# simonmeister/UnFlow

Measured on NVIDIA H100. Metric: frame-pairs/s at 384x1280 FlowNetC, higher is better.
Workload: dtype f32

## Files before the change

unflow_b200/csrc/tc_wgrad.cu:

```cuda
#include "tc_common.cuh"

namespace unflow {
namespace tcw {

using namespace unflow::tc;

constexpr int NTHREADS = 384;
constexpr int KP = 32;

struct WgradParams {
  int N, Hp, Wp;
  int TW, TH, TN;
  int tiles_x, tiles_y, tiles_n;
  int n_ptiles, kc, n_chunks;
  int R, C;
  int cgroups, vgroups;
  int r_blocks, c_blocks, taps, kw;
  int chunk;
  long long *dbg;
  int stride, stride_x, pad_t, pad_l;
  float *dw;
  long long pitch_r, pitch_t;
};

template <int BN>
struct Cfg {
  static constexpr int G_BYTES = BN * KP * 4;
  static constexpr int A_HI = 0;
  static constexpr int A_LO = A_HI + A_BYTES;
  static constexpr int B_HI = A_LO + A_BYTES;
  static constexpr int B_LO = B_HI + G_BYTES;
  static constexpr int SPLIT_BYTES = B_LO + G_BYTES;
  static constexpr int SPLIT_STAGES = 2;
  static constexpr int G_RAW = A_BYTES;
  static constexpr int RAW_BYTES = A_BYTES + G_BYTES;
  static constexpr int RAW0 = SPLIT_STAGES * SPLIT_BYTES;
  static constexpr int FIXED = RAW0 + 1024  + 256 ;
  static constexpr int RAW_STAGES = (SMEM_LIMIT - FIXED) / RAW_BYTES < 8 ? (SMEM_LIMIT - FIXED) / RAW_BYTES : 8;
  static constexpr int SMEM_BYTES = FIXED + RAW_STAGES * RAW_BYTES;
  static_assert(RAW_STAGES >= 3, "TMA at least two K blocks ahead of the split");
  static_assert(SMEM_BYTES <= SMEM_LIMIT, "over the shared memory of a block");
  static_assert(8 * (2 * RAW_STAGES + SPLIT_STAGES) <= 256, "barriers");
};

struct Item {
  int chunk, rb, cb;
};
__device__ __forceinline__ Item decode_item(const WgradParams &p, int it) {
  Item w;
  w.cb = it % p.c_blocks; it /= p.c_blocks;
  w.rb = it % p.r_blocks; it /= p.r_blocks;
  w.chunk = it;
  return w;
}
__device__ __forceinline__ int chunk_len(const WgradParams &p, int chunk) {
  const int k0 = chunk * p.kc;
  return (k0 + p.kc <= p.n_ptiles) ? p.kc : p.n_ptiles - k0;
}

template <int ROWS>
__device__ __forceinline__ void split_transpose(const float *raw, unsigned char *hi, unsigned char *lo, int row0, int ct) {
#pragma unroll
  for (int j = 0; j < ROWS * 8 / 128; ++j) {
    const int i = ct + 128 * j;
    const int r = row0 + i % ROWS, c = i / ROWS;
    const float *src = raw + (r >> 5) * 1024 + (4 * c) * 32 + (r & 31);
    const float4 v = make_float4(src[0], src[32], src[64], src[96]), h = tf32_hi4(v);
    const unsigned o = sw128_offset(r, 4 * c);
    *reinterpret_cast<float4 *>(hi + o) = h;
    *reinterpret_cast<float4 *>(lo + o) = sub4(v, h);
  }
}

template <int BN>
__global__ void __launch_bounds__(NTHREADS, 1)
tc_wgrad_kernel(const __grid_constant__ CUtensorMap mapP, const __grid_constant__ CUtensorMap mapG,
                const __grid_constant__ WgradParams p) {
  using C = Cfg<BN>;
  constexpr int R = BN / 2;
  constexpr int GROUPS = BN / 32;
  extern __shared__ unsigned char smem_raw[];
  const unsigned base = (s32(smem_raw) + 1023u) & ~1023u;
  unsigned char *gbase = smem_raw + (base - s32(smem_raw));
  const unsigned bars = base + C::RAW0 + C::RAW_STAGES * C::RAW_BYTES;
  auto raw_full = [&](int s) { return bars + 8u * s; };
  auto raw_empty = [&](int s) { return bars + 8u * (C::RAW_STAGES + s); };
  auto split_empty = [&](int s) { return bars + 8u * (2 * C::RAW_STAGES + s); };

  const int warp = __shfl_sync(0xffffffffu, threadIdx.x >> 5, 0), lane = threadIdx.x & 31;
  const int total_items = p.n_chunks * p.r_blocks * p.c_blocks;

  if (threadIdx.x == 0) {
    for (int s = 0; s < C::RAW_STAGES; ++s) {
      mbar_init(raw_full(s), 1);
      mbar_init(raw_empty(s), 8);
    }
    for (int s = 0; s < C::SPLIT_STAGES; ++s) mbar_init(split_empty(s), 8);
    asm volatile("fence.mbarrier_init.release.cluster;" ::: "memory");
    asm volatile("prefetch.tensormap [%0];" ::"l"(&mapP) : "memory");
    asm volatile("prefetch.tensormap [%0];" ::"l"(&mapG) : "memory");
  }
  __syncthreads();

  if (warp == 0) {
    int s = 0;
    unsigned ph = 0;
    long long t_wait = 0, t_all = clock64();
    for (int item = blockIdx.x; item < total_items; item += gridDim.x) {
      const Item w = decode_item(p, item);
      int gch[GROUPS], gdx[GROUPS], gdy[GROUPS];
#pragma unroll
      for (int j = 0; j < GROUPS; ++j) {
        const int v = w.cb * GROUPS + j;
        if (v < p.vgroups) {
          const int tap = v / p.cgroups, ky = tap / p.kw;
          gch[j] = (v - tap * p.cgroups) * 32; gdy[j] = ky - p.pad_t; gdx[j] = tap - ky * p.kw - p.pad_l;
        } else {
          gch[j] = p.cgroups * 32; gdx[j] = gdy[j] = 0;
        }
      }
      const int k0 = w.chunk * p.kc, klen = chunk_len(p, w.chunk);
      for (int kb = k0; kb < k0 + klen; ++kb) {
        int q = kb;
        const int px = (q % p.tiles_x) * p.TW; q /= p.tiles_x;
        const int py = (q % p.tiles_y) * p.TH; q /= p.tiles_y;
        const int pn = q * p.TN;
        { const long long t0 = clock64(); mbar_wait(raw_empty(s), ph ^ 1u); t_wait += clock64() - t0; }
        const unsigned st = base + C::RAW0 + s * C::RAW_BYTES;
        if (elect_one()) {
          mbar_expect_tx(raw_full(s), (unsigned)C::RAW_BYTES);
#pragma unroll
          for (int j = 0; j < BM / 32; ++j)
            tma_4d(st + j * 4096, &mapP, raw_full(s), w.rb * BM + 32 * j, px, py, pn);
#pragma unroll
          for (int j = 0; j < GROUPS; ++j)
            tma_4d(st + C::G_RAW + j * 4096, &mapG, raw_full(s), gch[j], p.stride_x * px + gdx[j],
                   p.stride * py + gdy[j], pn);
        }
        __syncwarp();
        if (++s == C::RAW_STAGES) { s = 0; ph ^= 1u; }
      }
    }
    if (p.dbg && blockIdx.x == 0 && lane == 0) { p.dbg[0] = t_wait; p.dbg[1] = clock64() - t_all; }
  } else if (warp >= 4) {
    const int cw = (warp >> 2) - 1;
    const int ct = threadIdx.x - 128 * (cw + 1);
    const int row0 = 64 * cw + 16 * (ct >> 5) + (lane >> 2);
    const int col0 = 2 * (lane & 3);
    unsigned n = 0;
    unsigned t_wait = 0, t_split = 0;
    const unsigned t_all = (unsigned)clock();
    auto split = [&](bool rows) {
      const unsigned rs = n % C::RAW_STAGES, rph = (n / C::RAW_STAGES) & 1u;
      const unsigned ss = n % C::SPLIT_STAGES, sph = (n / C::SPLIT_STAGES) & 1u;
      { const unsigned t0 = (unsigned)clock(); mbar_wait(raw_full(rs), rph); t_wait += (unsigned)clock() - t0; }
      { const unsigned t0 = (unsigned)clock(); mbar_wait(split_empty(ss), sph ^ 1u); t_split += (unsigned)clock() - t0; }
      const float *raw = reinterpret_cast<const float *>(gbase + C::RAW0 + rs * C::RAW_BYTES);
      unsigned char *sp = gbase + ss * C::SPLIT_BYTES;
      if (rows) split_transpose<64>(raw, sp + C::A_HI, sp + C::A_LO, 64 * cw, ct);
      split_transpose<BN / 2>(raw + C::G_RAW / 4, sp + C::B_HI, sp + C::B_LO, cw * (BN / 2), ct);
      __syncwarp();
      if (lane == 0) mbar_arrive(raw_empty(rs));
      fence_proxy_async();
      named_bar_sync(1, 256);
    };
    float sum[R], acc[R];
    for (int item = blockIdx.x; item < total_items; item += gridDim.x) {
      const Item w = decode_item(p, item);
      const int iters = chunk_len(p, w.chunk);
      if (w.rb * BM + 64 * cw >= p.R) {
        for (int it = 0; it < iters; ++it) {
          split(false);
          if (lane == 0) mbar_arrive(split_empty(n % C::SPLIT_STAGES));
          ++n;
        }
        continue;
      }
#pragma unroll
      for (int c = 0; c < R; ++c) sum[c] = 0.f;
      for (int c0 = 0; c0 < iters; c0 += p.chunk) {
        const int c1 = c0 + p.chunk < iters ? c0 + p.chunk : iters;
        for (int it = c0; it < c1; ++it) {
          split(true);
          const unsigned st = base + (n % C::SPLIT_STAGES) * C::SPLIT_BYTES;
          const unsigned long long a_hi = wgmma_desc_k128(st + C::A_HI + cw * (A_BYTES / 2));
          const unsigned long long a_lo = wgmma_desc_k128(st + C::A_LO + cw * (A_BYTES / 2));
          const unsigned long long b_hi = wgmma_desc_k128(st + C::B_HI), b_lo = wgmma_desc_k128(st + C::B_LO);
          fence_regs(acc);
          wgmma_fence();
#pragma unroll
          for (int k = 0; k < KP / 8; ++k) {
            const unsigned long long adv = (unsigned long long)(2 * k);
            Wgmma<BN>::mma(acc, a_lo + adv, b_hi + adv, (it - c0 | k) != 0);
            Wgmma<BN>::mma(acc, a_hi + adv, b_lo + adv, 1);
            Wgmma<BN>::mma(acc, a_hi + adv, b_hi + adv, 1);
          }
          wgmma_commit();
          wgmma_wait<1>();
          fence_regs(acc);
          __syncwarp();
          if (it > c0 && lane == 0) mbar_arrive(split_empty((n - 1) % C::SPLIT_STAGES));
          ++n;
        }
        wgmma_wait<0>();
        fence_regs(acc);
        __syncwarp();
        if (lane == 0) mbar_arrive(split_empty((n - 1) % C::SPLIT_STAGES));
#pragma unroll
        for (int c = 0; c < R; ++c) sum[c] += acc[c];
      }
#pragma unroll
      for (int h = 0; h < 2; ++h) {
        const int r = w.rb * BM + row0 + 8 * h;
        if (r >= p.R) continue;
#pragma unroll
        for (int j = 0; j < BN / 8; ++j) {
          const int col = 8 * j + col0;
          const int v = w.cb * GROUPS + col / 32;
          if (v >= p.vgroups) continue;
          const int tap = v / p.cgroups, c = (v - tap * p.cgroups) * 32 + (col & 31);
          float *dst = p.dw + (long long)r * p.pitch_r + (long long)tap * p.pitch_t + c;
          if (c < p.C) red_add_f32(dst, sum[4 * j + 2 * h]);
          if (c + 1 < p.C) red_add_f32(dst + 1, sum[4 * j + 2 * h + 1]);
        }
      }
    }
    if (p.dbg && blockIdx.x == 0 && threadIdx.x == 128) {
      p.dbg[2] = t_wait; p.dbg[3] = (unsigned)clock() - t_all; p.dbg[4] = t_split;
      p.dbg[5] = C::RAW_STAGES; p.dbg[6] = C::SPLIT_STAGES;
    }
  }
}

template <int BN>
static int launch(const CUtensorMap &mP, const CUtensorMap &mG, const WgradParams &p, cudaStream_t stream) {
  using C = Cfg<BN>;
  static bool attr_set = false;
  if (!attr_set) {
    cudaError_t e = cudaFuncSetAttribute(tc_wgrad_kernel<BN>, cudaFuncAttributeMaxDynamicSharedMemorySize, C::SMEM_BYTES);
    if (e != cudaSuccess) { set_error("tc_wgrad: cannot opt in to %d bytes of shared memory: %s", C::SMEM_BYTES, cudaGetErrorString(e)); return UNFLOW_ECUDA; }
    attr_set = true;
  }
  const long long total = (long long)p.n_chunks * p.r_blocks * p.c_blocks;
  const int grid = total < kNumSMs ? (int)total : kNumSMs;
  tc_wgrad_kernel<BN><<<grid, NTHREADS, C::SMEM_BYTES, stream>>>(mP, mG, p);
  count_launch();
  return check_launch("tc_wgrad_kernel");
}

static int launch_bn(int BN, const CUtensorMap &mP, const CUtensorMap &mG, const WgradParams &p, cudaStream_t stream) {
  if (BN == 128) return launch<128>(mP, mG, p, stream);
  if (BN == 64) return launch<64>(mP, mG, p, stream);
  return launch<32>(mP, mG, p, stream);
}

static void choose_box(WgradParams &p) {
  long long best = -1;
  for (int TW = 1; TW <= 32; TW *= 2)
    for (int TH = 1; TW * TH <= 32; TH *= 2) {
      const int TN = 32 / (TW * TH);
      const long long tiles = (long long)((p.Wp + TW - 1) / TW) * ((p.Hp + TH - 1) / TH) * ((p.N + TN - 1) / TN);
      if (best < 0 || tiles < best || (tiles == best && TW > p.TW)) {
        best = tiles; p.TW = TW; p.TH = TH; p.TN = TN;
      }
    }
  p.tiles_x = (p.Wp + p.TW - 1) / p.TW; p.tiles_y = (p.Hp + p.TH - 1) / p.TH; p.tiles_n = (p.N + p.TN - 1) / p.TN;
  p.n_ptiles = p.tiles_x * p.tiles_y * p.tiles_n;
}

static int make_plan(WgradParams &p, int &BN, int N, int Hp, int Wp, int R, int C, int stride, int kh, int kw,
                     int pad_t, int pad_l) {
  UNFLOW_REQUIRE(N > 0 && Hp > 0 && Wp > 0 && R > 0 && C > 0, "tc_wgrad: bad extents");
  UNFLOW_REQUIRE(stride == 1 || stride == 2, "tc_wgrad: stride must be 1 or 2");
  UNFLOW_REQUIRE(kh > 0 && kw > 0 && kh * kw <= 64, "tc_wgrad: at most 64 taps");
  p.N = N; p.Hp = Hp; p.Wp = Wp; p.R = R; p.C = C; p.chunk = g_chunk; p.dbg = g_dbg;
  p.taps = kh * kw; p.kw = kw; p.stride = p.stride_x = stride; p.pad_t = pad_t; p.pad_l = pad_l;
  choose_box(p);
  p.cgroups = (C + 31) / 32; p.vgroups = p.taps * p.cgroups;
  BN = p.vgroups >= 4 ? 128 : (p.vgroups >= 2 ? 64 : 32);
  p.r_blocks = (R + BM - 1) / BM; p.c_blocks = (p.vgroups + BN / 32 - 1) / (BN / 32);
  const long long tiles = (long long)p.r_blocks * p.c_blocks;
  long long want = (6ll * kNumSMs + tiles - 1) / tiles;
  if (want < 1) want = 1;
  int kc = (int)((p.n_ptiles + want - 1) / want);
  if (kc < 8) kc = p.n_ptiles < 8 ? p.n_ptiles : 8;
  p.kc = kc; p.n_chunks = (p.n_ptiles + kc - 1) / kc;
  UNFLOW_REQUIRE(tiles * p.n_chunks < (1ll << 30), "tc_wgrad: too many work items");
  return UNFLOW_OK;
}

}
}

using namespace unflow;

extern "C" int unflow_tc_wgrad_plan(int N, int Hp, int Wp, int R, int C, int stride, int kh, int kw, int pad_t,
                                    int pad_l, int *out) {
  tcw::WgradParams p{};
  int BN = 0;
  if (tcw::make_plan(p, BN, N, Hp, Wp, R, C, stride, kh, kw, pad_t, pad_l) || !out) return -1;
  const int v[15] = {p.TW, p.TH, p.TN, p.tiles_x, p.tiles_y, p.tiles_n, p.n_ptiles, p.kc, p.n_chunks, p.r_blocks,
                     p.c_blocks, BN, p.taps, p.cgroups, p.vgroups};
  for (int i = 0; i < 15; ++i) out[i] = v[i];
  return 15;
}

extern "C" int unflow_tc_wgrad(const float *P, int N, int Hp, int Wp, int R, long long p_pitch, const float *G,
                               int Hg, int Wg, int C, long long g_pitch, float *dw, long long pitch_r,
                               long long pitch_t, int stride, int kh, int kw, int pad_t, int pad_l, void *stream) {
  UNFLOW_REQUIRE(P && G && dw, "tc_wgrad: null pointer");
  UNFLOW_REQUIRE(Hg > 0 && Wg > 0, "tc_wgrad: bad extents");
  UNFLOW_REQUIRE(p_pitch % 4 == 0 && g_pitch % 4 == 0 && p_pitch >= R && g_pitch >= C,
                 "tc_wgrad: channel pitches must be multiples of 4 floats");
  UNFLOW_REQUIRE(((uintptr_t)P & 15) == 0 && ((uintptr_t)G & 15) == 0, "tc_wgrad: P and G must be 16-byte aligned");
  tcw::WgradParams p{};
  int BN = 0;
  int rc = tcw::make_plan(p, BN, N, Hp, Wp, R, C, stride, kh, kw, pad_t, pad_l);
  if (rc) return rc;
  p.dw = dw; p.pitch_r = pitch_r; p.pitch_t = pitch_t;
  CUtensorMap mP, mG;
  {
    cuuint64_t dims[4] = {(cuuint64_t)R, (cuuint64_t)Wp, (cuuint64_t)Hp, (cuuint64_t)N};
    cuuint64_t strides[3] = {(cuuint64_t)p_pitch * 4, (cuuint64_t)p_pitch * 4 * Wp, (cuuint64_t)p_pitch * 4 * Wp * Hp};
    cuuint32_t box[4] = {32, (cuuint32_t)p.TW, (cuuint32_t)p.TH, (cuuint32_t)p.TN};
    cuuint32_t estr[4] = {1, 1, 1, 1};
    rc = tc::encode(&mP, P, 4, dims, strides, box, estr, CU_TENSOR_MAP_SWIZZLE_NONE);
    if (rc) return rc;
  }
  {
    cuuint64_t dims[4] = {(cuuint64_t)C, (cuuint64_t)Wg, (cuuint64_t)Hg, (cuuint64_t)N};
    cuuint64_t strides[3] = {(cuuint64_t)g_pitch * 4, (cuuint64_t)g_pitch * 4 * Wg, (cuuint64_t)g_pitch * 4 * Wg * Hg};
    cuuint32_t box[4] = {32, (cuuint32_t)(p.TW * stride), (cuuint32_t)(p.TH * stride), (cuuint32_t)p.TN};
    cuuint32_t estr[4] = {1, (cuuint32_t)stride, (cuuint32_t)stride, 1};
    rc = tc::encode(&mG, G, 4, dims, strides, box, estr, CU_TENSOR_MAP_SWIZZLE_NONE);
    if (rc) return rc;
  }
  return tcw::launch_bn(BN, mP, mG, p, (cudaStream_t)stream);
}

extern "C" int unflow_tc_wgrad_window(const float *P, int N, int Ho, int Wo, int R, long long p_pitch,
                                      const float *xp, int H, int Wp, int Cp, float *dw, int kh, int stride,
                                      int pad_t, void *stream) {
  UNFLOW_REQUIRE(P && xp && dw, "tc_wgrad_window: null pointer");
  UNFLOW_REQUIRE(Cp == 4 || Cp == 8 || Cp == 16, "tc_wgrad_window: padded channel count must be 4, 8 or 16");
  UNFLOW_REQUIRE(p_pitch % 4 == 0 && p_pitch >= R, "tc_wgrad_window: bad pitch");
  UNFLOW_REQUIRE(((uintptr_t)P & 15) == 0 && ((uintptr_t)xp & 15) == 0, "tc_wgrad_window: pointers must be 16-byte aligned");
  UNFLOW_REQUIRE(H > 0 && Wp >= stride * (Wo - 1) + 8, "tc_wgrad_window: the padded row must hold the last 8-pixel window");
  const int win = 8 * Cp;
  tcw::WgradParams p{};
  int BN = 0;
  int rc = tcw::make_plan(p, BN, N, Ho, Wo, R, win, stride, kh, 1, pad_t, 0);
  if (rc) return rc;
  p.stride_x = 1;
  p.dw = dw; p.pitch_r = (long long)kh * win; p.pitch_t = win;
  CUtensorMap mP, mG;
  {
    cuuint64_t dims[4] = {(cuuint64_t)R, (cuuint64_t)Wo, (cuuint64_t)Ho, (cuuint64_t)N};
    cuuint64_t strides[3] = {(cuuint64_t)p_pitch * 4, (cuuint64_t)p_pitch * 4 * Wo, (cuuint64_t)p_pitch * 4 * Wo * Ho};
    cuuint32_t box[4] = {32, (cuuint32_t)p.TW, (cuuint32_t)p.TH, (cuuint32_t)p.TN};
    cuuint32_t estr[4] = {1, 1, 1, 1};
    rc = tc::encode(&mP, P, 4, dims, strides, box, estr, CU_TENSOR_MAP_SWIZZLE_NONE);
    if (rc) return rc;
  }
  {
    cuuint64_t dims[4] = {(cuuint64_t)win, (cuuint64_t)Wo, (cuuint64_t)H, (cuuint64_t)N};
    cuuint64_t strides[3] = {(cuuint64_t)stride * Cp * 4, (cuuint64_t)Wp * Cp * 4, (cuuint64_t)Wp * Cp * 4 * H};
    cuuint32_t box[4] = {32, (cuuint32_t)p.TW, (cuuint32_t)(p.TH * stride), (cuuint32_t)p.TN};
    cuuint32_t estr[4] = {1, 1, (cuuint32_t)stride, 1};
    rc = tc::encode(&mG, xp, 4, dims, strides, box, estr, CU_TENSOR_MAP_SWIZZLE_NONE);
    if (rc) return rc;
  }
  return tcw::launch_bn(BN, mP, mG, p, (cudaStream_t)stream);
}
```

Before: 114.8.

## Feed wgrad A operand from registers instead of split shared-memory tiles

The A (P) operand of the 3xTF32 weight-gradient WGMMA is now loaded directly from the swizzled raw TMA stage into registers, split into hi/lo in registers, and issued as register-source wgmma, removing the A split/transpose pass and its shared-memory stage. Raw-stage release moves to after the register loads, and commits are per K-step with double-buffered fragment sets so loads overlap the previous MMAs. Register budgets are rebalanced with setmaxnreg (producer warps shrink, consumers grow), and the P tensor map uses the default swizzle to match the new addressing. This risks register pressure and more per-element conversion work in the consumer warps, and the B-side indexing change must stay consistent with the G layout.

```diff
diff --git a/unflow_b200/csrc/tc_wgrad.cu b/unflow_b200/csrc/tc_wgrad.cu
--- a/unflow_b200/csrc/tc_wgrad.cu
+++ b/unflow_b200/csrc/tc_wgrad.cu
@@ -26,9 +26,7 @@
 template <int BN>
 struct Cfg {
   static constexpr int G_BYTES = BN * KP * 4;
-  static constexpr int A_HI = 0;
-  static constexpr int A_LO = A_HI + A_BYTES;
-  static constexpr int B_HI = A_LO + A_BYTES;
+  static constexpr int B_HI = 0;
   static constexpr int B_LO = B_HI + G_BYTES;
   static constexpr int SPLIT_BYTES = B_LO + G_BYTES;
   static constexpr int SPLIT_STAGES = 2;
@@ -58,14 +56,17 @@
   return (k0 + p.kc <= p.n_ptiles) ? p.kc : p.n_ptiles - k0;
 }
 
+constexpr int FRAG_SETS = 2;
+static_assert((KP / 8) % FRAG_SETS == 0 && FRAG_SETS <= KP / 8, "fragment sets per K block");
+
 template <int ROWS>
 __device__ __forceinline__ void split_transpose(const float *raw, unsigned char *hi, unsigned char *lo, int row0, int ct) {
 #pragma unroll
   for (int j = 0; j < ROWS * 8 / 128; ++j) {
     const int i = ct + 128 * j;
     const int r = row0 + i % ROWS, c = i / ROWS;
-    const float *src = raw + (r >> 5) * 1024 + (4 * c) * 32 + (r & 31);
-    const float4 v = make_float4(src[0], src[32], src[64], src[96]), h = tf32_hi4(v);
+    const float *src = raw + (r >> 5) * 1024 + (8 * (c >> 1) + (c & 1)) * 32 + (r & 31);
+    const float4 v = make_float4(src[0], src[64], src[128], src[192]), h = tf32_hi4(v);
     const unsigned o = sw128_offset(r, 4 * c);
     *reinterpret_cast<float4 *>(hi + o) = h;
     *reinterpret_cast<float4 *>(lo + o) = sub4(v, h);
@@ -102,6 +103,7 @@
   }
   __syncthreads();
 
+  if (warp < 4) setmaxnreg_dec<40>();
   if (warp == 0) {
     int s = 0;
     unsigned ph = 0;
@@ -143,35 +145,38 @@
     }
     if (p.dbg && blockIdx.x == 0 && lane == 0) { p.dbg[0] = t_wait; p.dbg[1] = clock64() - t_all; }
   } else if (warp >= 4) {
+    setmaxnreg_inc<232>();
     const int cw = (warp >> 2) - 1;
     const int ct = threadIdx.x - 128 * (cw + 1);
     const int row0 = 64 * cw + 16 * (ct >> 5) + (lane >> 2);
     const int col0 = 2 * (lane & 3);
     unsigned n = 0;
-    unsigned t_wait = 0, t_split = 0;
-    const unsigned t_all = (unsigned)clock();
-    auto split = [&](bool rows) {
+    long long t_wait = 0, t_split = 0, t_all = clock64();
+    auto split = [&]() {
       const unsigned rs = n % C::RAW_STAGES, rph = (n / C::RAW_STAGES) & 1u;
       const unsigned ss = n % C::SPLIT_STAGES, sph = (n / C::SPLIT_STAGES) & 1u;
-      { const unsigned t0 = (unsigned)clock(); mbar_wait(raw_full(rs), rph); t_wait += (unsigned)clock() - t0; }
-      { const unsigned t0 = (unsigned)clock(); mbar_wait(split_empty(ss), sph ^ 1u); t_split += (unsigned)clock() - t0; }
+      { const long long t0 = clock64(); mbar_wait(raw_full(rs), rph); t_wait += clock64() - t0; }
+      { const long long t0 = clock64(); mbar_wait(split_empty(ss), sph ^ 1u); t_split += clock64() - t0; }
       const float *raw = reinterpret_cast<const float *>(gbase + C::RAW0 + rs * C::RAW_BYTES);
       unsigned char *sp = gbase + ss * C::SPLIT_BYTES;
-      if (rows) split_transpose<64>(raw, sp + C::A_HI, sp + C::A_LO, 64 * cw, ct);
       split_transpose<BN / 2>(raw + C::G_RAW / 4, sp + C::B_HI, sp + C::B_LO, cw * (BN / 2), ct);
-      __syncwarp();
-      if (lane == 0) mbar_arrive(raw_empty(rs));
       fence_proxy_async();
       named_bar_sync(1, 256);
+      return raw;
     };
     float sum[R], acc[R];
+    unsigned a_hi[FRAG_SETS][4], a_lo[FRAG_SETS][4];
     for (int item = blockIdx.x; item < total_items; item += gridDim.x) {
       const Item w = decode_item(p, item);
       const int iters = chunk_len(p, w.chunk);
       if (w.rb * BM + 64 * cw >= p.R) {
         for (int it = 0; it < iters; ++it) {
-          split(false);
-          if (lane == 0) mbar_arrive(split_empty(n % C::SPLIT_STAGES));
+          split();
+          __syncwarp();
+          if (lane == 0) {
+            mbar_arrive(raw_empty(n % C::RAW_STAGES));
+            mbar_arrive(split_empty(n % C::SPLIT_STAGES));
+          }
           ++n;
         }
         continue;
@@ -180,32 +185,47 @@
       for (int c = 0; c < R; ++c) sum[c] = 0.f;
       for (int c0 = 0; c0 < iters; c0 += p.chunk) {
         const int c1 = c0 + p.chunk < iters ? c0 + p.chunk : iters;
+        int pending = -1;
         for (int it = c0; it < c1; ++it) {
-          split(true);
-          const unsigned st = base + (n % C::SPLIT_STAGES) * C::SPLIT_BYTES;
-          const unsigned long long a_hi = wgmma_desc_k128(st + C::A_HI + cw * (A_BYTES / 2));
-          const unsigned long long a_lo = wgmma_desc_k128(st + C::A_LO + cw * (A_BYTES / 2));
+          const float *a = split() + (row0 >> 5) * 1024;
+          const int ch = row0 & 31;
+          const unsigned rs = n % C::RAW_STAGES, ss = n % C::SPLIT_STAGES;
+          const unsigned st = base + ss * C::SPLIT_BYTES;
           const unsigned long long b_hi = wgmma_desc_k128(st + C::B_HI), b_lo = wgmma_desc_k128(st + C::B_LO);
-          fence_regs(acc);
-          wgmma_fence();
 #pragma unroll
           for (int k = 0; k < KP / 8; ++k) {
+            unsigned (&hi)[4] = a_hi[k % FRAG_SETS], (&lo)[4] = a_lo[k % FRAG_SETS];
+            wgmma_wait<FRAG_SETS - 1>();
+            fence_regs(acc);
+            if (k == FRAG_SETS - 1) {
+              __syncwarp();
+              if (pending >= 0 && lane == 0) mbar_arrive(split_empty(pending));
+            }
+#pragma unroll
+            for (int e = 0; e < 4; ++e) {
+              const float x = a[sw128_offset(8 * k + 2 * (lane & 3) + (e >> 1), ch + 8 * (e & 1)) / 4];
+              const float h = tf32_rna_fast(x);
+              hi[e] = __float_as_uint(h);
+              lo[e] = __float_as_uint(x - h);
+            }
+            if (k == KP / 8 - 1) {
+              __syncwarp();
+              if (lane == 0) mbar_arrive(raw_empty(rs));
+            }
+            wgmma_fence();
             const unsigned long long adv = (unsigned long long)(2 * k);
-            Wgmma<BN>::mma(acc, a_lo + adv, b_hi + adv, (it - c0 | k) != 0);
-            Wgmma<BN>::mma(acc, a_hi + adv, b_lo + adv, 1);
-            Wgmma<BN>::mma(acc, a_hi + adv, b_hi + adv, 1);
+            Wgmma<BN>::mma_rs(acc, lo, b_hi + adv, (it - c0 | k) != 0);
+            Wgmma<BN>::mma_rs(acc, hi, b_lo + adv, 1);
+            Wgmma<BN>::mma_rs(acc, hi, b_hi + adv, 1);
+            wgmma_commit();
           }
-          wgmma_commit();
-          wgmma_wait<1>();
-          fence_regs(acc);
-          __syncwarp();
-          if (it > c0 && lane == 0) mbar_arrive(split_empty((n - 1) % C::SPLIT_STAGES));
+          pending = ss;
           ++n;
         }
         wgmma_wait<0>();
         fence_regs(acc);
         __syncwarp();
-        if (lane == 0) mbar_arrive(split_empty((n - 1) % C::SPLIT_STAGES));
+        if (lane == 0) mbar_arrive(split_empty(pending));
 #pragma unroll
         for (int c = 0; c < R; ++c) sum[c] += acc[c];
       }
@@ -226,7 +246,7 @@
       }
     }
     if (p.dbg && blockIdx.x == 0 && threadIdx.x == 128) {
-      p.dbg[2] = t_wait; p.dbg[3] = (unsigned)clock() - t_all; p.dbg[4] = t_split;
+      p.dbg[2] = t_wait; p.dbg[3] = clock64() - t_all; p.dbg[4] = t_split;
       p.dbg[5] = C::RAW_STAGES; p.dbg[6] = C::SPLIT_STAGES;
     }
   }
@@ -324,7 +344,7 @@
     cuuint64_t strides[3] = {(cuuint64_t)p_pitch * 4, (cuuint64_t)p_pitch * 4 * Wp, (cuuint64_t)p_pitch * 4 * Wp * Hp};
     cuuint32_t box[4] = {32, (cuuint32_t)p.TW, (cuuint32_t)p.TH, (cuuint32_t)p.TN};
     cuuint32_t estr[4] = {1, 1, 1, 1};
-    rc = tc::encode(&mP, P, 4, dims, strides, box, estr, CU_TENSOR_MAP_SWIZZLE_NONE);
+    rc = tc::encode(&mP, P, 4, dims, strides, box, estr);
     if (rc) return rc;
   }
   {
@@ -359,7 +379,7 @@
     cuuint64_t strides[3] = {(cuuint64_t)p_pitch * 4, (cuuint64_t)p_pitch * 4 * Wo, (cuuint64_t)p_pitch * 4 * Wo * Ho};
     cuuint32_t box[4] = {32, (cuuint32_t)p.TW, (cuuint32_t)p.TH, (cuuint32_t)p.TN};
     cuuint32_t estr[4] = {1, 1, 1, 1};
-    rc = tc::encode(&mP, P, 4, dims, strides, box, estr, CU_TENSOR_MAP_SWIZZLE_NONE);
+    rc = tc::encode(&mP, P, 4, dims, strides, box, estr);
     if (rc) return rc;
   }
   {
```

Result: faster. 118.4 (median of 6 runs) (+3.1%).
